# The-Learning-And-Vision-Atelier-LAVA/BUFFER

Hardware: AMD Instinct MI355X
Metric: registration pairs/sec (higher is better)
Workload: dtype f32

## Files before the change

buffer_amd/_lib.py:

```python
import ctypes as C
import os

_HERE = os.path.dirname(os.path.abspath(__file__))
LIB_PATH = os.environ.get("BUF_LIB_PATH") or os.path.join(_HERE, "libbuffer_hip.so")

BUF_OK = 0


class BufferHipError(RuntimeError):
    pass


class buf_grid_t(C.Structure):
    _fields_ = [
        ("ws", C.c_void_p), ("ws_bytes", C.c_size_t),
        ("ns", C.c_int), ("nb", C.c_int),
        ("cells_per_elem", C.c_int64),
        ("radius", C.c_float),
        ("supports", C.c_void_p),
        ("desc", C.c_void_p), ("s_off", C.c_void_p), ("table", C.c_void_p),
        ("sorted", C.c_void_p), ("order", C.c_void_p), ("scan_tmp", C.c_void_p),
    ]


# ... 102 lines not shown
    "buf_sc2_ws_bytes": (_sz, [_vp, _i, _i]),
    "buf_sc2_batched": (_i, [_vp, _vp, _vp, _vp, _vp, _vp, _i, C.c_double, C.c_double, C.c_double, _i, _i, C.c_double, _i, _i,
                             _vp, _vp, _vp, _vp, _vp, _vp, _vp, _vp, _sz, _vp]),
    "buf_clique_ws_bytes": (_sz, [_vp, _i, _i, _i]),
    "buf_clique_batched": (_i, [_vp, _vp, _vp, _vp, _vp, _vp, _i, C.c_double, C.c_double, C.c_double, C.c_double, _i, _i, C.c_double, _i,
                                _i, _vp, _vp, _vp, _vp, _vp, _vp, _vp, _vp, _vp, _vp, _vp, _sz, _vp]),
    "buf_voxel_map_bytes": (_sz, [_i, _i, _i64]),
    "buf_voxel_map_ws_bytes": (_sz, [_i, _i, _i64]),
    "buf_voxel_map_build": (_i, [C.POINTER(buf_voxel_map_t), _vp, _vp, _vp, _i, C.c_double, C.c_double, _i64, _vp, _sz, _vp, _sz, _vp]),
    "buf_voxel_map_export": (_i, [C.POINTER(buf_voxel_map_t), _i, _vp, _vp, _vp, _vp, _vp, _vp]),
    "buf_vgicp_ws_bytes": (_sz, [_i, _i]),
    "buf_vgicp_batched": (_i, [C.POINTER(buf_voxel_map_t), _vp, _vp, _vp, _vp, _i, _i, _vp, _i, C.c_double, C.c_double, _vp, _vp, _vp,
                               _vp, _vp, _vp, _sz, _vp]),
    "buf_match_metrics":(_i, [_vp, _vp, _vp, _i, _i, _vp, _vp, _f, _f, _f, _vp, _vp, _vp]),
    "buf_row_linear": (_i, [_vp, _i, _i, _i, _vp, _vp, _i, _vp, _vp]),
    "buf_segment_instance_norm_ws_bytes": (_sz, [_i, _i]),
    "buf_segment_instance_norm": (_i, [_vp, _i, _i, _vp, _i, _f, _vp, _vp, _sz, _vp]),
    "buf_descriptor_head": (_i, [_vp, _i, _vp, _vp, _vp, _vp]),
    "buf_cost_volume_net": (_i, [_vp, _vp, _i, _vp, _vp, _vp, _vp]),
    "buf_cost_volume_net_gather": (_i, [_vp, _i, _vp, _vp, _i, _vp, _vp, _vp, _vp]),
    "buf_cost_volume_net_w24": (_i, [_vp, _vp, _i, _vp, _vp, _vp, _vp, _vp]),
    "buf_cost_volume_net_w24_gather": (_i, [_vp, _i, _vp, _vp, _i, _vp, _vp, _vp, _vp, _vp]),
    "buf_cost_volume_net_split_safe_w24": (_i, [_vp, _vp, _i, _vp, _vp, _i, _vp, _vp, _vp, _vp, _vp, _vp, _vp, _vp, _vp]),
    "buf_hypotheses_score": (_i, [_vp, _vp, _vp, _vp, _vp, _i, _i, _f, _vp, _vp, _vp, _vp, _vp, _vp]),
    "buf_ransac_ws_bytes": (_sz, [_i]),
    "buf_ransac_kabsch": (_i, [_vp, _vp, _vp, _i, _i, C.c_uint64, _f, _f, _vp, _vp, _vp, _sz, _vp]),
    "buf_ransac_masked_ws_bytes": (_sz, [_i, _i]),
    "buf_ransac_kabsch_masked": (_i, [_vp, _vp, _vp, _i, _i, C.c_uint64, _f, _f, _vp, _vp, _vp, _sz, _vp]),
    "buf_post_refine": (_i, [_vp, _vp, _vp, _i, _f, _i, _vp, _vp, _vp]),
    "buf_recover_poses_ws_bytes": (_sz, [_i, _i, _i]),
    "buf_recover_poses_batched": (_i, [_vp, _vp, _vp, _vp, _vp, _vp, _i, _vp, _i, _f, _i, _f, _f, _f, _i, _vp, _vp, _sz, _vp]),
}


def exported_symbols():
    return sorted(_SIGNATURES)


def lib():
    global _lib
    if _lib is None:
        if not os.path.exists(LIB_PATH):
            raise BufferHipError(
                f"{LIB_PATH} is missing: build it with `python -m buffer_amd.build` "
                "(hipcc --offload-arch=gfx950). buffer_amd has no CPU fallback.")
        import torch
# ... 14 lines not shown
```

buffer_amd/csrc/buffer_hip.hip:

```cpp
#include <stdlib.h>
#include "core.hip"
#include "radius.hip"
#include "icp.hip"
#include "pairstats.hip"
#include "posegraph.hip"
#include "metrics.hip"
#include "subsample.hip"
#include "pointops.hip"
#include "vn.hip"
#include "voxelize.hip"
#include "registration.hip"
#include "convnet.hip"
#include "convnet_h3.hip"
#include "costnet_h3.hip"
#include "preprocess.hip"
#include "convnet_wg.hip"
#include "convnet_w24.hip"
#include "convnet_w24k.hip"
#include "convnet_w24p.hip"
#include "convnet_w24a.hip"
#include "costnet.hip"
#include "costnet_w24.hip"
#include "split_safe.hip"
#include "fpfh.hip"
#include "fgr.hip"
#include "sc2.hip"
#include "clique.hip"
#include "vgicp.hip"
```

buffer_amd/csrc/costnet.hip:

```cpp
#include "common.h"
#include <type_traits>

#define CV_THREADS 256
#define CV_BUF 20480
#define CV_LAYERS 10
#define CV_C32 36
#define CV_C64 68
#define CV_C128 132

typedef float cvx4 __attribute__((ext_vector_type(4)));

#define CV_SCHED_TAIL(NMFMA, NMEM)                                                      \
    _Pragma("unroll") for (int i_ = 0; i_ < (NMFMA); i_++) {                            \
        __builtin_amdgcn_sched_group_barrier(0x008, 1, 0);                              \
        __builtin_amdgcn_sched_group_barrier(0x006, 4, 0);                              \
        __builtin_amdgcn_sched_group_barrier(0x120, ((NMEM) + (NMFMA) - 1) / (NMFMA), 0); \
    }
typedef const __attribute__((address_space(1))) cvx4* cv_gptr;

struct CostNetParams {
    const float* wt[CV_LAYERS];
    const float* bias[CV_LAYERS];
    const long long* s_rows;
    const long long* t_rows;
// ... 240 lines not shown
        int j = lq - (r0 + t);
        j = j < 0 ? j + 20 : j;
        const cvx4 sv = *reinterpret_cast<const cvx4*>(SM + (kq * 20 + j) * CV_C32 + c4 * 4);
        const cvx4 tv = *reinterpret_cast<const cvx4*>(TB + pos * CV_C32 + c4 * 4);
        float* d = X + (kq * 32 + c4 * 4) * CW_CSX + t * CW_RSX + lq;
#pragma unroll
        for (int q = 0; q < 4; q++) d[q * CW_CSX] = fmaxf(sv[q] + tv[q], 0.f);
    }
}

#ifdef CV_STAMP
__device__ long long* cv_stamp_ptr;
#define CV_STAMP_AT(SLOT) if (threadIdx.x == 0) cv_stamp_ptr[(size_t)blockIdx.x * 16 + (SLOT)] = __builtin_amdgcn_s_memtime();
#else
#define CV_STAMP_AT(SLOT)
#endif

#define CW_CS5 72
template <int C, int CS, int USED>
__device__ __forceinline__ void cw24_zero_spare(float* __restrict__ map);
template <int HIN, int RS, int CS, int NTX, int TYPM, int CIN, int RSO, int CSO>
__device__ __forceinline__ void cw24_layer(float* __restrict__ map, const float* __restrict__ wt, const float* __restrict__ bias, int pair, int t);

template <bool W24 = false>
__device__ __forceinline__ void cost_net_body(const float* __restrict__ s_eq, const float* __restrict__ t_eq, const CostNetParams& P,
                                              float* __restrict__ ind_out, float* __restrict__ lds, const float* const* f24 = nullptr)
{
    float* bufA = lds;
    float* bufB = lds;
    float* SP = bufB + CVA_SP;
    float* TP = bufB + CVA_TP;
    float* SM = bufB + CVA_SM;
    float* TB = bufB + CVA_TB;
    const int match = blockIdx.x;
    const int tid = threadIdx.x, lane = tid & (WAVE - 1), li = lane & 15, lk = lane >> 4;
    const int w = __builtin_amdgcn_readfirstlane(tid / WAVE);
    {
        const float* a = s_eq + (P.s_rows ? (size_t)P.s_rows[match] * P.row_floats + P.skip_floats : (size_t)match * 3200);
        const float* b = t_eq + (P.t_rows ? (size_t)P.t_rows[match] * P.row_floats + P.skip_floats : (size_t)match * 3200);
        for (int i = tid; i < 800; i += CV_THREADS) {
            const int c = i / 25, rem = i - c * 25, k = rem / 5, l0 = (rem - k * 5) * 4;
            const cvx4 sv = __builtin_nontemporal_load(reinterpret_cast<const cvx4*>(a + c * P.chan_floats + rem * 4));
            const cvx4 tv = __builtin_nontemporal_load(reinterpret_cast<const cvx4*>(b + c * P.chan_floats + rem * 4));
#pragma unroll
            for (int q = 0; q < 4; q++) {
                const int l = l0 + q;
                SP[(k * 24 + l + 2) * CV_C32 + c] = sv[q];
// ... 11 lines not shown
        int ms = w * 16 + li, mt = ms;
        ms = ms < 60 ? ms : 59;
        mt = mt < 54 ? mt : 53;
        SLoader LS;
        LS.base = SP + ((ms / 20) * 24 + ms % 20) * CV_C32 + lk * 4;
        TLoader LT;
        LT.base = TP + ((mt / 18) * 20 + mt % 18) * CV_C32 + lk * 4;
        cvx4 accS[1][2] = { { (cvx4){ 0.f, 0.f, 0.f, 0.f }, (cvx4){ 0.f, 0.f, 0.f, 0.f } } };
        cvx4 accT[1][2] = { { (cvx4){ 0.f, 0.f, 0.f, 0.f }, (cvx4){ 0.f, 0.f, 0.f, 0.f } } };
        cv_gemm_static<1, 2, 4, 30>(accS, LS, P.wt[0] + (size_t)lane * 4, 2);
        cv_gemm_static<1, 2, 4, 18>(accT, LT, P.wt[0] + (size_t)30 * 2 * 256 + (size_t)lane * 4, 2);
#pragma unroll
        for (int u = 0; u < 2; u++)
#pragma unroll
            for (int r = 0; r < 4; r++) {
                const int m = w * 16 + lk * 4 + r;
                if (m < 60) SM[m * CV_C32 + u * 16 + li] = accS[0][u][r];
                if (m < 54) TB[m * CV_C32 + u * 16 + li] = b0v[u] - accT[0][u][r];
            }
    }
    __syncthreads();
    CV_STAMP_AT(1)

    {
        int lane_ = threadIdx.x & (WAVE - 1);
        asm volatile("" : "+v"(lane_));
        const int li_ = lane_ & 15, lk_ = lane_ >> 4;
        const int p_ = w & 1, kh = w >> 1;
        float* XC = bufB + CVA_XC;
        constexpr unsigned KSTEP = 16u * CW_CSX;
        const __amdgpu_buffer_rsrc_t rs = wg_weights(P.wt[1]);
        const unsigned wp = (unsigned)p_ * (96 * 512) + (unsigned)(12 * kh) * 512;
        const unsigned lofs = lane_ * 16;
        unsigned RA[3][4];
        {
            const unsigned base = (unsigned)(size_t)(__attribute__((address_space(3))) const float*)XC + (unsigned)(12 * kh) * KSTEP;
#pragma unroll
            for (int a = 0; a < 4; a++) RA[0][a] = RA[1][a] = RA[2][a] = base + 4u * (unsigned)(lk_ * CW_CSX + (2 * (li_ >> 3) + a) * CW_RSX + 2 * (li_ & 7));
        }
        const float* bl = kh ? nullptr : P.bias[1] + p_ * 32 + lk_ * 4;
        wgf4 W[2][2];
        wg_first_weights<2, 0, 2>(rs, wp, lofs, 512, W);
        wgf4* slot = reinterpret_cast<wgf4*>(bufB + CVA_XCH) + (size_t)p_ * 8 * WAVE + lane_;
        wgf4 Yown[2][2][3][2][2];
#pragma unroll
        for (int j = 0; j < 4; j++) {
            form_rows_cm(XC, SM, TB, 4 * j);
// ... 12 lines not shown
            }
        }
        __syncthreads();
#pragma unroll
        for (int jj = 0; jj < 2; jj++)
#pragma unroll
            for (int n = 0; n < 2; n++)
                cw_store_tile<18, 2, 16, CW_CS1, false>(Yown[jj][n][0], 2 * kh + jj, 2 * p_ + n, bufA, li_, lk_);
        __syncthreads();
        CV_STAMP_AT(2)
    }
    bool f24_2 = false, f24_4 = false, f24_6 = false;
    if constexpr (W24) { f24_2 = f24[0] != nullptr; f24_4 = f24[1] != nullptr; f24_6 = f24[2] != nullptr; }
    if (W24 && f24_2) {
        if constexpr (W24) {
            cw24_zero_spare<64, CW_CS1, 256>(bufA);
            __syncthreads();
            cw24_layer<16, 16, CW_CS1, 4, 4, 64, 14, CW_CS2>(bufA, f24[0], P.bias[2], w & 1, w >> 1);
        }
    } else
        cw_layer<16, 16, CW_CS1, 2, 64, 2, 2, 0, 14, CW_CS2, false>(bufA, P.wt[2], P.bias[2], w & 1, 2 * (w >> 1));
    __syncthreads();
    CV_STAMP_AT(3)
    cw_layer<14, 14, CW_CS2, 2, 64, 2, 2, 1, 12, CW_CS3, false>(bufA, P.wt[3], P.bias[3], w, 0);
    __syncthreads();
    CV_STAMP_AT(4)
    if (W24 && f24_4) {
        if constexpr (W24) {
            cw24_zero_spare<128, CW_CS3, 144>(bufA);
            __syncthreads();
            cw24_layer<12, 12, CW_CS3, 3, 5, 128, 12, CW_CS3>(bufA, f24[1], P.bias[4], w, 0);
        }
    } else
        cw_layer<12, 12, CW_CS3, 3, 128, 2, 2, 0, 12, CW_CS3, false>(bufA, P.wt[4], P.bias[4], w, 0);
    __syncthreads();
    CV_STAMP_AT(5)
    if (W24 && f24_6) {
        if constexpr (W24) {
            cw_layer<10, 12, CW_CS3, 4, 128, 1, 1, 0, 8, CW_CS5, false>(bufA, P.wt[5], P.bias[5], w, 0);
            __syncthreads();
            CV_STAMP_AT(6)
            cw_layer<8, 8, CW_CS5, 3, 64, 1, 1, 0, 0, CV_C64, true>(bufA, f24[2], P.bias[6], w, 0);
        }
    } else {
        cw_layer<10, 12, CW_CS3, 4, 128, 1, 1, 0, 0, CV_C64, true>(bufA, P.wt[5], P.bias[5], w, 0);
        __syncthreads();
        CV_STAMP_AT(6)
// ... 134 lines not shown
```

buffer_amd/csrc/split_safe.hip:

```cpp
#include "common.h"

extern "C" int buf_cylindrical_net_split_safe_form(const float* x, int npatch, const void* const* wt_split_host, const float* const* wt_wg_host,
                                                   const float* const* bias_host, const int* cin_host, const int* cout_host, const int* relu_host,
                                                   int form, const float* head_params, float* y_or_equi, float* desc, int* status_dev,
                                                   int* flags_ws, void* stream)
{
    BUF_REQUIRE(npatch >= 0, BUF_EINVAL, "buf_cylindrical_net_split_safe: npatch=%d", npatch);
    if (npatch == 0) return BUF_OK;
    BUF_REQUIRE(x && y_or_equi && flags_ws && wt_split_host && wt_wg_host && bias_host && cin_host && cout_host && relu_host, BUF_EINVAL,
                "buf_cylindrical_net_split_safe: null argument");
    BUF_REQUIRE(!head_params || desc, BUF_EINVAL, "buf_cylindrical_net_split_safe: head without desc");
    BUF_REQUIRE(form >= BUF_CYL_FORM_DEFAULT && form <= BUF_CYL_FORM_PASS_SPLIT, BUF_EINVAL,
                "buf_cylindrical_net_split_safe: form=%d (-1: the library's default, 0: K split, 1: pass split)", form);
    if (int rc = buf_cylindrical_net_wg_flags(cin_host, cout_host, relu_host)) return rc;
    hipStream_t s = (hipStream_t)stream;
    BUF_CHECK_HIP(hipMemsetAsync(flags_ws, 0, sizeof(int) * (size_t)npatch, s));
    int relu_split[WG_LAYERS];
    for (int l = 0; l < WG_LAYERS; l++) relu_split[l] = wg_f24_flagged(relu_host[l]) ? (relu_host[l] & 1) : relu_host[l];
    int rc = h3_launch(x, npatch, wt_split_host, bias_host, cin_host, cout_host, relu_split, head_params ? nullptr : y_or_equi, head_params,
                       desc, head_params ? y_or_equi : nullptr, status_dev, stream, flags_ws);
    if (rc) return rc;
    rc = wg_launch(x, npatch, wt_wg_host, bias_host, cin_host, cout_host, relu_host, y_or_equi, flags_ws, stream, form);
    if (rc) return rc;
    if (head_params) {
// ... 58 lines not shown
    if (rc) return rc;
    return cost_net_launch(s_eq, t_eq, m, wt_f32_host, bias_f32_host, s_rows, t_rows, ele_n, ind_out, stream, "buf_cost_volume_net_split_safe", flags_ws);
}

extern "C" int buf_cost_volume_net_split_safe_w24(const float* s_eq, const float* t_eq, int ele_n, const long long* s_rows, const long long* t_rows,
                                                  int m, const void* const* wt_split_host, const float* const* bias_split_host,
                                                  const float* const* wt_f32_host, const float* const* bias_f32_host, const float* const* f24_host,
                                                  float* ind_out, int* status_dev, int* flags_ws, void* stream)
{
    BUF_REQUIRE(m >= 0, BUF_EINVAL, "buf_cost_volume_net_split_safe_w24: m=%d", m);
    if (m == 0) return BUF_OK;
    BUF_REQUIRE(s_eq && t_eq && wt_split_host && bias_split_host && wt_f32_host && bias_f32_host && f24_host && ind_out && flags_ws, BUF_EINVAL,
                "buf_cost_volume_net_split_safe_w24: null argument");
    BUF_REQUIRE((s_rows == nullptr) == (t_rows == nullptr), BUF_EINVAL, "buf_cost_volume_net_split_safe_w24: one row list without the other");
    BUF_REQUIRE(!s_rows || ele_n == 7, BUF_EINVAL, "buf_cost_volume_net_split_safe_w24: ele_n=%d (the kernels are built for ele_n = 7)", ele_n);
    hipStream_t s = (hipStream_t)stream;
    BUF_CHECK_HIP(hipMemsetAsync(flags_ws, 0, sizeof(int) * (size_t)m, s));
    int rc = cost_net_h3_launch(s_eq, t_eq, m, wt_split_host, bias_split_host, s_rows, t_rows, ele_n, ind_out, status_dev, stream,
                                "buf_cost_volume_net_split_safe_w24", flags_ws);
    if (rc) return rc;
    return cost_net_w24_launch(s_eq, t_eq, m, wt_f32_host, bias_f32_host, f24_host, s_rows, t_rows, ele_n, ind_out, stream,
                               "buf_cost_volume_net_split_safe_w24", flags_ws);
}
```

buffer_amd/ops.py:

```python
import ctypes as C
import time
import os
import numpy as np
import torch

from . import _lib
from ._lib import buf_grid_t, check


def _stream():
    return C.c_void_p(torch.cuda.current_stream().cuda_stream)


def _dev(t, dtype, what):
    if not isinstance(t, torch.Tensor) or not t.is_cuda:
        raise _lib.BufferHipError(f"{what}: expected a tensor in device memory (buffer_amd has no CPU path)")
    if t.dtype != dtype:
        t = t.to(dtype)
    return t.contiguous()


def _ptr(t):
    return C.c_void_p(t.data_ptr()) if t is not None else C.c_void_p(0)

# ... 1078 lines not shown
        f24 = COST_F24_DEFAULT
    if f24 is True:
        f24 = 'all'
    if f24 is False:
        f24 = 'off'
    if f24 not in COST_F24_PARTS:
        raise ValueError(f"f24 = {f24!r}: one of 'all', 'l2', 'l4', 'l6', 'off'")
    return COST_F24_PARTS[f24]


def cost_f24_filters(layers, parts):
    sets = []
    for l in (2, 4, 6):
        if l not in parts:
            sets.append(None)
            continue
        w = layers[l][0]
        assert tuple(w.shape[2:]) == (3, 1, 3), w.shape
        w2d = np.ascontiguousarray(w[:, :, :, 0, :])
        sets.append(winograd_tile_weights(w2d, ng=1) if l == 6 else winograd_f24_tile_weights(w2d))
    return sets


class CostVolumeNet:

    def __init__(self, layers, device, f24=None):
        assert len(layers) == 10
        self.parts = cost_f24_parts(f24)
        self.wt24 = [None if a is None else torch.from_numpy(a).to(device) for a in cost_f24_filters(layers, self.parts)]
        self._fp = (C.c_void_p * 3)(*[None if t is None else t.data_ptr() for t in self.wt24])
        self.wt, self.bias = [], []
        for i, (w, b) in enumerate(layers):
            cout, cin = w.shape[0], w.shape[1]
            b = np.asarray(b, np.float32)
            if i == 0:
                assert tuple(w.shape) == (32, 32, 3, 3, 3), w.shape
                tiled = np.concatenate([mfma_tile_weights(m, lk_major=True) for m in separate_cost_layer0(w)])
                self.wt.append(torch.from_numpy(tiled).to(device))
                self.bias.append(torch.from_numpy(np.ascontiguousarray(b)).to(device))
                continue
            if i == 1:
                assert tuple(w.shape) == (64, 32, 3, 3, 3), w.shape
                w2d = np.ascontiguousarray(np.transpose(w, (0, 3, 1, 2, 4)).reshape(64, 96, 3, 3))
                self.wt.append(torch.from_numpy(winograd_tile_weights(w2d, ng=_lib.lib().buf_cost_winograd_group(1))).to(device))
                self.bias.append(torch.from_numpy(np.ascontiguousarray(b)).to(device))
                continue
            if 2 <= i <= 5:
                assert tuple(w.shape[2:]) == (3, 1, 3), w.shape
                tiled = winograd_tile_weights(np.ascontiguousarray(w[:, :, :, 0, :]), ng=_lib.lib().buf_cost_winograd_group(i))
                self.wt.append(torch.from_numpy(tiled).to(device))
                self.bias.append(torch.from_numpy(np.ascontiguousarray(b)).to(device))
                continue
            wt = np.transpose(w, (2, 3, 4, 1, 0)).reshape(-1, cout)
            if i == 9:
                wt = np.concatenate([wt, np.zeros((wt.shape[0], 32 - cout), np.float32)], 1)
                b = np.concatenate([b, np.zeros(32 - cout, np.float32)])
            self.wt.append(torch.from_numpy(mfma_tile_weights(np.ascontiguousarray(wt, dtype=np.float32), lk_major=True)).to(device))
            self.bias.append(torch.from_numpy(np.ascontiguousarray(b)).to(device))
        self._wp = (C.c_void_p * 10)(*[t.data_ptr() for t in self.wt])
        self._bp = (C.c_void_p * 10)(*[t.data_ptr() for t in self.bias])

    def __call__(self, s_eq, t_eq):
        L = _lib.lib()
        s_eq, t_eq = s_eq.contiguous(), t_eq.contiguous()
        m = s_eq.shape[0]
        out = torch.empty((m,), dtype=torch.float32, device=s_eq.device)
        if self.parts:
            check(L.buf_cost_volume_net_w24(_ptr(s_eq), _ptr(t_eq), m, self._wp, self._bp, self._fp, _ptr(out), _stream()),
                  "buf_cost_volume_net_w24")
            return out
        check(L.buf_cost_volume_net(_ptr(s_eq), _ptr(t_eq), m, self._wp, self._bp, _ptr(out), _stream()),
              "buf_cost_volume_net")
        return out

    def gathered(self, equi, s_rows, t_rows):
        L = _lib.lib()
        equi = _dev(equi, torch.float32, "CostVolumeNet.gathered")
        if equi.dim() != 4 or tuple(equi.shape[1:]) != (32, 7, 20):
            raise _lib.BufferHipError(f"CostVolumeNet.gathered: expected [rows,32,7,20] maps, got {tuple(equi.shape)}")
        s_rows, t_rows = _dev(s_rows, torch.int64, "s_rows"), _dev(t_rows, torch.int64, "t_rows")
        m = int(s_rows.shape[0])
        out = torch.empty((m,), dtype=torch.float32, device=equi.device)
        if self.parts:
            check(L.buf_cost_volume_net_w24_gather(_ptr(equi), 7, _ptr(s_rows), _ptr(t_rows), m, self._wp, self._bp, self._fp, _ptr(out),
                                                   _stream()), "buf_cost_volume_net_w24_gather")
            return out
        check(L.buf_cost_volume_net_gather(_ptr(equi), 7, _ptr(s_rows), _ptr(t_rows), m, self._wp, self._bp, _ptr(out), _stream()),
              "buf_cost_volume_net_gather")
        return out


class CostVolumeNetSplit:

    def __init__(self, layers, device, f24=None):
        assert len(layers) == 10
        self.parts = cost_f24_parts(f24)
        mats = []
        w0 = layers[0][0]
        assert tuple(w0.shape) == (32, 32, 3, 3, 3), w0.shape
        ws, wt = separate_cost_layer0(w0)
        mats.append((np.transpose(ws.reshape(15, 32, 32), (2, 1, 0)), 2))
        mats.append((np.transpose(wt.reshape(9, 32, 32), (2, 1, 0)), 2))
        w1 = layers[1][0]
        assert tuple(w1.shape) == (64, 32, 3, 3, 3), w1.shape
        mats.append((np.transpose(w1, (0, 3, 1, 2, 4)).reshape(64, 96, 9), 2))
        for i in range(2, 9):
            w = layers[i][0]
            assert tuple(w.shape[2:]) == (3, 1, 3), w.shape
            mats.append((np.ascontiguousarray(w[:, :, :, 0, :]).reshape(w.shape[0], w.shape[1], 9), 2 if i < 7 else 1))
        w9 = layers[9][0]
        assert tuple(w9.shape) == (20, 32, 2, 1, 2), w9.shape
        mats.append((np.ascontiguousarray(w9[:, :, :, 0, :]).reshape(20, 32, 4), 1))
        self.wt = [torch.from_numpy(split_tile_gemm(m, nt).view(np.int16)).to(device) for m, nt in mats]
        self.bias = []
        for i, (_, b) in enumerate(layers):
            b = np.asarray(b, np.float32)
            if i == 9:
                b = np.concatenate([b, np.zeros(32 - b.shape[0], np.float32)])
            self.bias.append(torch.from_numpy(np.ascontiguousarray(b)).to(device))
        self.status = torch.zeros(1, dtype=torch.int32, device=device)
        self._wp = (C.c_void_p * 11)(*[t.data_ptr() for t in self.wt])
        self._bp = (C.c_void_p * 10)(*[t.data_ptr() for t in self.bias])
        self.safe = not os.environ.get('BUF_SPLIT_UNSAFE')
        self.f32 = CostVolumeNet(layers, device, f24=f24) if self.safe else None
        self.last_flags = None

    def _safe(self, s_eq, t_eq, s_rows, t_rows, m, dev):
        L = _lib.lib()
        out = torch.empty((m,), dtype=torch.float32, device=dev)
        self.last_flags = torch.empty((max(m, 1),), dtype=torch.int32, device=dev)
        if self.parts:
            check(L.buf_cost_volume_net_split_safe_w24(_ptr(s_eq), _ptr(t_eq), 7, _ptr(s_rows), _ptr(t_rows), m, self._wp, self._bp, self.f32._wp,
                                                       self.f32._bp, self.f32._fp, _ptr(out), _ptr(self.status), _ptr(self.last_flags), _stream()),
                  "buf_cost_volume_net_split_safe_w24")
            return out
        check(L.buf_cost_volume_net_split_safe(_ptr(s_eq), _ptr(t_eq), 7, _ptr(s_rows), _ptr(t_rows), m, self._wp, self._bp, self.f32._wp,
                                               self.f32._bp, _ptr(out), _ptr(self.status), _ptr(self.last_flags), _stream()),
              "buf_cost_volume_net_split_safe")
        return out

    def __call__(self, s_eq, t_eq):
        L = _lib.lib()
        s_eq, t_eq = s_eq.contiguous(), t_eq.contiguous()
        m = s_eq.shape[0]
        if self.safe:
            return self._safe(s_eq, t_eq, None, None, m, s_eq.device)
        out = torch.empty((m,), dtype=torch.float32, device=s_eq.device)
        check(L.buf_cost_volume_net_split(_ptr(s_eq), _ptr(t_eq), m, self._wp, self._bp, _ptr(out), _ptr(self.status), _stream()),
              "buf_cost_volume_net_split")
        return out

    def gathered(self, equi, s_rows, t_rows):
        L = _lib.lib()
# ... 21 lines not shown
```

buffer_amd/registration.py:

```python
import numpy as np

from . import ops
from .patch_embedder import _fold_bn


class CostVolume:

    def __init__(self, W, device, azi_n=20, arith='f32', f24=None):
        if arith not in ('f32', 'split'):
            raise ValueError(f"cnn_arith must be 'f32' or 'split', got {arith!r}")
        if azi_n != 20:
            raise NotImplementedError(f'CostVolume: the fused kernel is built for azi_n = 20 (got {azi_n})')
        self.azi_n = azi_n
        p = 'Inlier.conv.ops'
        layers = []
        for i, bn in ((0, 1), (3, 4), (6, 7), (9, 10), (12, 13), (15, 16), (18, 19), (21, 22), (24, 25)):
            layers.append(_fold_bn(W[f'{p}.{i}.weight'], W[f'{p}.{i}.bias'], W[f'{p}.{bn}.running_mean'], W[f'{p}.{bn}.running_var']))
        layers.append((np.asarray(W[f'{p}.27.weight'], np.float32), np.asarray(W[f'{p}.27.bias'], np.float32)))
        self.fused = ops.CostVolumeNetSplit(layers, device, f24=f24) if arith == 'split' else ops.CostVolumeNet(layers, device, f24=f24)

    def __call__(self, d1, d2):
        if tuple(d1.shape[1:]) != (32, 5, 20) or d1.shape != d2.shape:
            raise ValueError(f'CostVolume: expected two [M,32,5,20] maps, got {tuple(d1.shape)} and {tuple(d2.shape)}')
        return self.fused(d1, d2)

    def gathered(self, equi, s_rows, t_rows):
        return self.fused.gathered(equi, s_rows, t_rows)
```

include/buffer_hip.h:

```cpp
#ifndef BUFFER_HIP_H
#define BUFFER_HIP_H
#include <stddef.h>
#include <stdint.h>
#ifdef __cplusplus
extern "C" {
#endif

#define BUF_OK            0
#define BUF_EINVAL       -1
#define BUF_EHIP         -2
#define BUF_EWORKSPACE   -3
#define BUF_ECAPACITY    -4
#define BUF_ENODEVICE    -5

const char* buf_last_error(void);
int         buf_version(void);
int         buf_device_count(void);
#define BUF_TIMED_GRID_QUERY 0
#define BUF_TIMED_CYL_NET    1
#define BUF_TIMED_COST_NET   2
#define BUF_TIMED_SELECT_PATCHES 3
#define BUF_TIMED_PATCH_VOXELIZE 4
#define BUF_TIMED_FPS            5
#define BUF_TIMED_NN1            6
// ... 150 lines not shown
                                       const float* head_params, float* y_or_equi, float* desc, int* status_dev, int* flags_ws, void* stream);

int     buf_cylindrical_net_split_safe_form(const float* x, int npatch, const void* const* wt_split_host, const float* const* wt_wg_host,
                                            const float* const* bias_host, const int* cin_host, const int* cout_host, const int* relu_host,
                                            int form, const float* head_params, float* y_or_equi, float* desc, int* status_dev, int* flags_ws,
                                            void* stream);
int     buf_cylindrical_net_split_safe_all(const float* x, int npatch, const void* const* wt_split_host, const float* const* wt_wg_host,
                                           const float* const* bias_host, const int* cin_host, const int* cout_host, const int* relu_host,
                                           const float* const* wt24_host, const float* head_params, float* y_or_equi, float* desc,
                                           int* status_dev, int* flags_ws, void* stream);

int     buf_descriptor_head(const float* y, int npatch, const float* params, float* desc, float* equi, void* stream);

int     buf_cost_winograd_group(int layer);
int     buf_cost_volume_net(const float* s_eq, const float* t_eq, int m, const float* const* wt_host,
                            const float* const* bias_host, float* ind_out, void* stream);
int     buf_cost_volume_net_gather(const float* equi, int ele_n, const long long* s_rows, const long long* t_rows, int m,
                                   const float* const* wt_host, const float* const* bias_host, float* ind_out, void* stream);
int     buf_cost_volume_net_w24(const float* s_eq, const float* t_eq, int m, const float* const* wt_host, const float* const* bias_host,
                                const float* const* f24_host, float* ind_out, void* stream);
int     buf_cost_volume_net_w24_gather(const float* equi, int ele_n, const long long* s_rows, const long long* t_rows, int m,
                                       const float* const* wt_host, const float* const* bias_host, const float* const* f24_host,
                                       float* ind_out, void* stream);

long long buf_split_gemm_count(int cout, int cin, int ntaps, int nt);
int     buf_split_tile_gemm(const float* w_host, int cout, int cin, int ntaps, int nt, unsigned short* out_host);
int     buf_cost_volume_net_split(const float* s_eq, const float* t_eq, int m, const void* const* wt_host,
                                  const float* const* bias_host, float* ind_out, int* status_dev, void* stream);
int     buf_cost_volume_net_split_gather(const float* equi, int ele_n, const long long* s_rows, const long long* t_rows, int m,
                                         const void* const* wt_host, const float* const* bias_host, float* ind_out,
                                         int* status_dev, void* stream);
int     buf_cost_volume_net_split_safe(const float* s_eq, const float* t_eq, int ele_n, const long long* s_rows, const long long* t_rows,
                                       int m, const void* const* wt_split_host, const float* const* bias_split_host,
                                       const float* const* wt_f32_host, const float* const* bias_f32_host, float* ind_out,
                                       int* status_dev, int* flags_ws, void* stream);
int     buf_cost_volume_net_split_safe_w24(const float* s_eq, const float* t_eq, int ele_n, const long long* s_rows, const long long* t_rows,
                                           int m, const void* const* wt_split_host, const float* const* bias_split_host,
                                           const float* const* wt_f32_host, const float* const* bias_f32_host, const float* const* f24_host,
                                           float* ind_out, int* status_dev, int* flags_ws, void* stream);

int     buf_hypotheses_score(const float* ind, const float* ss_kpts, const float* tt_kpts, const float* ss_R,
                             const float* tt_R, int m, int azi_n, float inlier_th, float* R_out, float* t_out,
                             int* inlier_num, int* best_out, unsigned char* best_mask, void* stream);
size_t  buf_ransac_ws_bytes(int nhyp);
int     buf_ransac_kabsch(const float* src, const float* tgt, const int* corr, int ncorr, int nhyp,
                          unsigned long long seed, float max_dist, float edge_similarity, float* T_out,
                          int* info_out, void* ws, size_t ws_bytes, void* stream);
size_t  buf_ransac_masked_ws_bytes(int m, int nhyp);
int     buf_ransac_kabsch_masked(const float* src, const float* tgt, const unsigned char* mask, int m, int nhyp,
                                 unsigned long long seed, float max_dist, float edge_similarity, float* T_out,
                                 int* info_out, void* ws, size_t ws_bytes, void* stream);
int     buf_post_refine(const float* T_init, const float* src, const float* tgt, int m, float inlier_threshold,
                        int iters, float* T_out, int* info_out, void* stream);
size_t  buf_recover_poses_ws_bytes(int m_total, int nb, int nhyp);
int     buf_recover_poses_batched(const float* ind, const float* ss_kpts, const float* tt_kpts, const float* ss_R, const float* tt_R,
                                  const int* seg_host, int nb, const unsigned long long* seeds_host, int azi_n, float inlier_th,
                                  int nhyp, float max_dist, float edge_similarity, float refine_threshold, int refine_iters,
                                  float* poses_out, void* ws, size_t ws_bytes, void* stream);

size_t  buf_voxel_downsample_ws_bytes(int n, int64_t max_cells);
int     buf_voxel_downsample(const void* pts, const void* normals, int is_f64, int n, double voxel_size, double* out_pts,
                             double* out_normals, int* out_m_host, int64_t max_cells, void* ws, size_t ws_bytes, void* stream);
// ... 127 lines not shown
```

Measured before the change: 175.3.

## Add Winograd F(2x4) paths for cost-volume layers 1 and 3

Adds a w24b cost-net kernel that computes layer 1 (a 3x3x3 conv folded into a 2D conv over 96 channels, with the input plane formed per depth slice) and layer 3 with Winograd F(2x4) tiles. Layer 3 also gets an F(2x2) tail for the leftover rows. It becomes the default when f24 is unset, and the goal is fewer multiply-adds in these direct convolutions. The cost is extra transform arithmetic, extra LDS plane rebuilding and syncs, register pressure, and small floating-point differences.

Result: faster. 177.3, median of 6 (+1.1%).

```diff
diff --git a/buffer_amd/_lib.py b/buffer_amd/_lib.py
--- a/buffer_amd/_lib.py
+++ b/buffer_amd/_lib.py
@@ -148,6 +148,9 @@
     "buf_cost_volume_net_w24": (_i, [_vp, _vp, _i, _vp, _vp, _vp, _vp, _vp]),
     "buf_cost_volume_net_w24_gather": (_i, [_vp, _i, _vp, _vp, _i, _vp, _vp, _vp, _vp, _vp]),
     "buf_cost_volume_net_split_safe_w24": (_i, [_vp, _vp, _i, _vp, _vp, _i, _vp, _vp, _vp, _vp, _vp, _vp, _vp, _vp, _vp]),
+    "buf_cost_volume_net_w24b": (_i, [_vp, _vp, _i, _vp, _vp, _vp, _vp, _vp]),
+    "buf_cost_volume_net_w24b_gather": (_i, [_vp, _i, _vp, _vp, _i, _vp, _vp, _vp, _vp, _vp]),
+    "buf_cost_volume_net_split_safe_w24b": (_i, [_vp, _vp, _i, _vp, _vp, _i, _vp, _vp, _vp, _vp, _vp, _vp, _vp, _vp, _vp]),
     "buf_hypotheses_score": (_i, [_vp, _vp, _vp, _vp, _vp, _i, _i, _f, _vp, _vp, _vp, _vp, _vp, _vp]),
     "buf_ransac_ws_bytes": (_sz, [_i]),
     "buf_ransac_kabsch": (_i, [_vp, _vp, _vp, _i, _i, C.c_uint64, _f, _f, _vp, _vp, _vp, _sz, _vp]),
diff --git a/buffer_amd/csrc/buffer_hip.hip b/buffer_amd/csrc/buffer_hip.hip
--- a/buffer_amd/csrc/buffer_hip.hip
+++ b/buffer_amd/csrc/buffer_hip.hip
@@ -21,6 +21,7 @@
 #include "convnet_w24a.hip"
 #include "costnet.hip"
 #include "costnet_w24.hip"
+#include "costnet_w24b.hip"
 #include "split_safe.hip"
 #include "fpfh.hip"
 #include "fgr.hip"
diff --git a/buffer_amd/csrc/costnet.hip b/buffer_amd/csrc/costnet.hip
--- a/buffer_amd/csrc/costnet.hip
+++ b/buffer_amd/csrc/costnet.hip
@@ -286,7 +286,11 @@
 template <int HIN, int RS, int CS, int NTX, int TYPM, int CIN, int RSO, int CSO>
 __device__ __forceinline__ void cw24_layer(float* __restrict__ map, const float* __restrict__ wt, const float* __restrict__ bias, int pair, int t);
 
-template <bool W24 = false>
+__device__ __forceinline__ void cw24b_layer1(float* __restrict__ lds, const float* __restrict__ wt, const float* __restrict__ bias, int w);
+__device__ __forceinline__ void cw24b_layer3(float* __restrict__ map, const float* __restrict__ wt24, const float* __restrict__ wt22,
+                                             const float* __restrict__ bias, int w);
+
+template <bool W24 = false, bool W24B = false>
 __device__ __forceinline__ void cost_net_body(const float* __restrict__ s_eq, const float* __restrict__ t_eq, const CostNetParams& P,
                                               float* __restrict__ ind_out, float* __restrict__ lds, const float* const* f24 = nullptr)
 {
@@ -344,7 +348,14 @@
     __syncthreads();
     CV_STAMP_AT(1)
 
-    {
+    bool f24_1 = false, f24_3 = false;
+    if constexpr (W24B) { f24_1 = f24[3] != nullptr; f24_3 = f24[4] != nullptr; }
+    if (W24B && f24_1) {
+        if constexpr (W24B) {
+            cw24b_layer1(lds, f24[3], P.bias[1], w);
+            CV_STAMP_AT(2)
+        }
+    } else {
         int lane_ = threadIdx.x & (WAVE - 1);
         asm volatile("" : "+v"(lane_));
         const int li_ = lane_ & 15, lk_ = lane_ >> 4;
@@ -403,7 +414,10 @@
         cw_layer<16, 16, CW_CS1, 2, 64, 2, 2, 0, 14, CW_CS2, false>(bufA, P.wt[2], P.bias[2], w & 1, 2 * (w >> 1));
     __syncthreads();
     CV_STAMP_AT(3)
-    cw_layer<14, 14, CW_CS2, 2, 64, 2, 2, 1, 12, CW_CS3, false>(bufA, P.wt[3], P.bias[3], w, 0);
+    if (W24B && f24_3) {
+        if constexpr (W24B) cw24b_layer3(bufA, f24[4], P.wt[3], P.bias[3], w);
+    } else
+        cw_layer<14, 14, CW_CS2, 2, 64, 2, 2, 1, 12, CW_CS3, false>(bufA, P.wt[3], P.bias[3], w, 0);
     __syncthreads();
     CV_STAMP_AT(4)
     if (W24 && f24_4) {
diff --git a/buffer_amd/csrc/costnet_w24b.hip b/buffer_amd/csrc/costnet_w24b.hip
--- /dev/null
+++ b/buffer_amd/csrc/costnet_w24b.hip
@@ -0,0 +1,281 @@
+#include "common.h"
+
+#ifndef CWB_RS1
+#define CWB_RS1 24
+#define CWB_CS1 450
+#endif
+static_assert(32 * CWB_CS1 <= CVA_SM, "the plane ends in front of the layer-0 maps");
+static_assert(17 * CWB_RS1 + 4 * 3 + 6 <= CWB_CS1 && CWB_RS1 % 2 == 0 && CWB_CS1 % 2 == 0, "the last window stays inside the channel; ds_read_b64");
+static_assert(64 * CW_CS1 <= CV_BUF, "layer 1's output map");
+
+struct CostNetW24BParams {
+    CostNetParams P;
+    const float* f24[5];
+};
+
+__device__ __forceinline__ void cw24b_form_plane(float* __restrict__ X, const float* __restrict__ SM, const float* __restrict__ TB, int kq)
+{
+    for (int i = threadIdx.x; i < 324 * 8; i += CV_THREADS) {
+        const int c4 = i & 7, pos = i >> 3, n = pos / 18, lq = pos - n * 18;
+        int j = lq - n;
+        j = j < 0 ? j + 20 : j;
+        const cvx4 sv = *reinterpret_cast<const cvx4*>(SM + (kq * 20 + j) * CV_C32 + c4 * 4);
+        const cvx4 tv = *reinterpret_cast<const cvx4*>(TB + (kq * 18 + lq) * CV_C32 + c4 * 4);
+        float* d = X + c4 * 4 * CWB_CS1 + n * CWB_RS1 + lq;
+#pragma unroll
+        for (int q = 0; q < 4; q++) d[q * CWB_CS1] = fmaxf(sv[q] + tv[q], 0.f);
+    }
+}
+
+template <unsigned KSTEP>
+__device__ __forceinline__ void cw24b_round_add(unsigned (&RA)[4], __amdgpu_buffer_rsrc_t rs, unsigned wp, unsigned wp_after, unsigned lofs4, unsigned lofs2,
+                                                int niter, unsigned pstride, const float* __restrict__ bias_lane, wgf4 (&W4)[2][2], wgf2 (&W2)[2][2],
+                                                wgf4 (&Y)[2][2][4])
+{
+    using std::integral_constant;
+    wgf2 D[2][6];
+    wgf4 bv[2];
+#pragma unroll
+    for (int n = 0; n < 2; n++) bv[n] = bias_lane ? *reinterpret_cast<const wgf4*>(bias_lane + n * 16) : (wgf4){ 0.f, 0.f, 0.f, 0.f };
+    wgf4 acc[2][6];
+    float zero = 0.f;
+    asm volatile("" : "+v"(zero));
+    auto run = [&](auto ic) __attribute__((always_inline)) {
+        constexpr int I = decltype(ic)::value;
+        constexpr int INEXT = I == 3 ? 0 : I + 1;
+#pragma unroll
+        for (int n = 0; n < 2; n++)
+#pragma unroll
+            for (int j = 0; j < 6; j++) acc[n][j] = (I == 1 && j == 1) ? bv[n] : (wgf4){ zero, zero, zero, zero };
+        constexpr int ICHAIN = (INEXT != 0 && wg_chains(I)) ? INEXT : -1;
+        w24_pass<I, wg_chains(I - 1), ICHAIN, KSTEP>(RA, rs, wp + I * pstride, INEXT == 0 ? wp_after : wp + (I + 1) * pstride, lofs4, lofs2, niter, W4, W2, acc, D);
+        __builtin_amdgcn_sched_barrier(0);
+#pragma unroll
+        for (int n = 0; n < 2; n++) {
+            wgf4 f[4];
+#pragma unroll
+            for (int r = 0; r < 4; r++) {
+                const float p = acc[n][1][r] + acc[n][2][r], q = acc[n][1][r] - acc[n][2][r];
+                const float t = acc[n][3][r] + acc[n][4][r], d = acc[n][3][r] - acc[n][4][r];
+                f[0][r] = acc[n][0][r] + p + t;
+                f[1][r] = __builtin_fmaf(2.f, d, q);
+                f[2][r] = __builtin_fmaf(4.f, t, p);
+                f[3][r] = __builtin_fmaf(8.f, d, q) + acc[n][5][r];
+            }
+#pragma unroll
+            for (int v = 0; v < 4; v++) {
+                if constexpr (I <= 2) Y[n][0][v] += f[v];
+                if constexpr (I == 1) Y[n][1][v] += f[v];
+                if constexpr (I >= 2) Y[n][1][v] -= f[v];
+                if constexpr (I <= 2) asm volatile("" : "+v"(Y[n][0][v]));
+                if constexpr (I >= 1) asm volatile("" : "+v"(Y[n][1][v]));
+            }
+        }
+    };
+    run(integral_constant<int, 0>{});
+    run(integral_constant<int, 1>{});
+    run(integral_constant<int, 2>{});
+    run(integral_constant<int, 3>{});
+}
+
+__device__ __forceinline__ void cw24b_layer1(float* __restrict__ lds, const float* __restrict__ wt, const float* __restrict__ bias, int w)
+{
+    float* X = lds + CVA_XC;
+    const float* SM = lds + CVA_SM;
+    const float* TB = lds + CVA_TB;
+    constexpr unsigned KSTEP = 16u * CWB_CS1;
+    int lane = threadIdx.x & (WAVE - 1);
+    asm volatile("" : "+v"(lane));
+    const int lk = lane >> 4;
+    const int pair = w & 1, t = w >> 1;
+    unsigned RA[4];
+    {
+        const unsigned base = (unsigned)(size_t)(__attribute__((address_space(3))) const float*)X;
+        const int li = lane & 15, ty = 4 * t + (li >> 2), tx = li & 3;
+#pragma unroll
+        for (int a = 0; a < 4; a++) RA[a] = base + 4u * (unsigned)(lk * CWB_CS1 + (2 * ty + a) * CWB_RS1 + 4 * tx);
+    }
+    const __amdgpu_buffer_rsrc_t rs = wg_weights(wt);
+    const unsigned pstride = 24u * W24_WSTRIDE;
+    const unsigned wp0 = (unsigned)pair * 4 * pstride;
+    const unsigned lofs4 = lane * 16, lofs2 = lane * 8;
+    const float* bv = bias + (2 * pair) * 16 + lk * 4;
+    wgf4 W4[2][2];
+    wgf2 W2[2][2];
+#pragma unroll
+    for (int n = 0; n < 2; n++)
+#pragma unroll
+        for (int k = 0; k < 2; k++) {
+            W4[n][k] = wg_ldw(rs, wp0 + k * W24_WSTRIDE + n * 256, lofs4);
+            W2[n][k] = w24_ldw2(rs, wp0 + k * W24_WSTRIDE + 512 + n * 128, lofs2);
+        }
+    wgf4 Y[2][2][4];
+    {
+        float zero = 0.f;
+        asm volatile("" : "+v"(zero));
+#pragma unroll
+        for (int q = 0; q < 16; q++) Y[q >> 3][(q >> 2) & 1][q & 3] = (wgf4){ zero, zero, zero, zero };
+    }
+#pragma unroll 1
+    for (int k = 0; k < 3; k++) {
+        cw24b_form_plane(X, SM, TB, k);
+        __syncthreads();
+        const unsigned wp = wp0 + 8u * k * W24_WSTRIDE;
+        cw24b_round_add<KSTEP>(RA, rs, wp, k < 2 ? wp + 8u * W24_WSTRIDE : wp0, lofs4, lofs2, 2, pstride, k == 0 ? bv : nullptr, W4, W2, Y);
+        __syncthreads();
+    }
+    int lane_s = threadIdx.x & (WAVE - 1);
+    asm volatile("" : "+v"(lane_s));
+    const int li = lane_s & 15, ty = 4 * t + (li >> 2), tx = li & 3;
+#pragma unroll
+    for (int n = 0; n < 2; n++) {
+        float* p = lds + ((2 * pair + n) * 16 + (lane_s >> 4) * 4) * CW_CS1 + 2 * ty * 16 + 4 * tx;
+#pragma unroll
+        for (int u = 0; u < 2; u++)
+#pragma unroll
+            for (int r = 0; r < 4; r++)
+                *reinterpret_cast<wgf4*>(p + r * CW_CS1 + u * 16) = (wgf4){ fmaxf(Y[n][u][0][r], 0.f), fmaxf(Y[n][u][1][r], 0.f), fmaxf(Y[n][u][2][r], 0.f), fmaxf(Y[n][u][3][r], 0.f) };
+    }
+    __syncthreads();
+}
+
+__device__ __forceinline__ void cw24b_layer3(float* __restrict__ map, const float* __restrict__ wt24, const float* __restrict__ wt22,
+                                             const float* __restrict__ bias, int w)
+{
+    constexpr int HIN = 14, RS = 14, CS = CW_CS2, NTX = 3, TYPM = 5, CIN = 64, RSO = 12, CSO = CW_CS3, k4 = CIN / 4;
+    static_assert((2 * (TYPM - 1) + 3) * RS + 4 * (NTX - 1) + 6 <= HIN * RS && RS % 2 == 0 && CS % 2 == 0, "the last F(2x4) window ends inside its row");
+    constexpr unsigned KSTEP = 16u * CS;
+    int lane = threadIdx.x & (WAVE - 1);
+    asm volatile("" : "+v"(lane));
+    const int lk = lane >> 4;
+    const unsigned base = (unsigned)(size_t)(__attribute__((address_space(3))) const float*)map;
+    unsigned RA[4];
+    {
+        const int li = lane & 15, q = li / NTX;
+        int ty = q, tx = li - q * NTX;
+        if (q >= TYPM) { ty = 0; tx = 0; }
+#pragma unroll
+        for (int a = 0; a < 4; a++) RA[a] = base + 4u * (unsigned)(lk * CS + (2 * ty + a) * RS + 4 * tx);
+    }
+    const unsigned lofs4 = lane * 16, lofs2 = lane * 8;
+    const float* bv = bias + (2 * w) * 16 + lk * 4;
+    wgf4 Y[2][2][4];
+    {
+        const __amdgpu_buffer_rsrc_t rs = wg_weights(wt24);
+        const unsigned pstride = (unsigned)(k4 * W24_WSTRIDE);
+        const unsigned wp = (unsigned)w * 4 * pstride;
+        wgf4 W4[2][2];
+        wgf2 W2[2][2];
+#pragma unroll
+        for (int n = 0; n < 2; n++)
+#pragma unroll
+            for (int k = 0; k < 2; k++) {
+                W4[n][k] = wg_ldw(rs, wp + k * W24_WSTRIDE + n * 256, lofs4);
+                W2[n][k] = w24_ldw2(rs, wp + k * W24_WSTRIDE + 512 + n * 128, lofs2);
+            }
+        w24_round<false, KSTEP>(RA, rs, wp, wp, lofs4, lofs2, k4 >> 2, pstride, bv, W4, W2, Y);
+    }
+    wgf4 Y2[2][3][2][2];
+    {
+        unsigned RB[3][4];
+        const int li = lane & 15, q = li / 6;
+        int ty = 4 + q, tx = li - q * 6;
+        if (q >= 2) { ty = 0; tx = 0; }
+#pragma unroll
+        for (int a = 0; a < 4; a++) RB[0][a] = RB[1][a] = RB[2][a] = base + 4u * (unsigned)(lk * CS + (2 * ty + a) * RS + 2 * tx);
+        const __amdgpu_buffer_rsrc_t rs = wg_weights(wt22);
+        const unsigned wp = (unsigned)w * (CIN * 2 * 256);
+        wgf4 W[2][2];
+        wg_first_weights<2, 0, 2>(rs, wp, lofs4, 512, W);
+        wg_round<2, 0, 1, KSTEP, true>(RB, rs, wp, wp, lofs4, k4 >> 2, 512, (unsigned)(k4 * 512), bv, W, Y2);
+    }
+    __syncthreads();
+    int lane_s = threadIdx.x & (WAVE - 1);
+    asm volatile("" : "+v"(lane_s));
+    const int li = lane_s & 15;
+    {
+        const int q = li / NTX, tx = li - q * NTX;
+        if (q < TYPM) {
+#pragma unroll
+            for (int n = 0; n < 2; n++) {
+                float* p = map + ((2 * w + n) * 16 + (lane_s >> 4) * 4) * CSO + 2 * q * RSO + 4 * tx;
+#pragma unroll
+                for (int u = 0; u < 2; u++)
+#pragma unroll
+                    for (int r = 0; r < 4; r++)
+                        *reinterpret_cast<wgf4*>(p + r * CSO + u * RSO) = (wgf4){ fmaxf(Y[n][u][0][r], 0.f), fmaxf(Y[n][u][1][r], 0.f), fmaxf(Y[n][u][2][r], 0.f), fmaxf(Y[n][u][3][r], 0.f) };
+            }
+        }
+    }
+    if (li >= 6 && li < 12) {
+#pragma unroll
+        for (int n = 0; n < 2; n++) {
+            float* p = map + ((2 * w + n) * 16 + (lane_s >> 4) * 4) * CSO + 10 * RSO + 2 * (li - 6);
+#pragma unroll
+            for (int u = 0; u < 2; u++)
+#pragma unroll
+                for (int r = 0; r < 4; r++)
+                    *reinterpret_cast<wgf2*>(p + r * CSO + u * RSO) = (wgf2){ fmaxf(Y2[n][0][u][0][r], 0.f), fmaxf(Y2[n][0][u][1][r], 0.f) };
+        }
+    }
+}
+
+__global__ void __launch_bounds__(CV_THREADS, 2) k_cost_net_w24b(const float* __restrict__ s_eq, const float* __restrict__ t_eq, CostNetW24BParams Q,
+                                                             float* __restrict__ ind_out)
+{
+    extern __shared__ float lds[];
+    cost_net_body<true, true>(s_eq, t_eq, Q.P, ind_out, lds, Q.f24);
+}
+
+__global__ void __launch_bounds__(CV_THREADS, 2) k_cost_net_w24b_rerun(const float* __restrict__ s_eq, const float* __restrict__ t_eq, CostNetW24BParams Q,
+                                                                   float* __restrict__ ind_out)
+{
+    extern __shared__ float lds[];
+    if (Q.P.only_if[blockIdx.x] == 0) return;
+    cost_net_body<true, true>(s_eq, t_eq, Q.P, ind_out, lds, Q.f24);
+}
+
+static int cost_net_w24b_launch(const float* s_eq, const float* t_eq, int m, const float* const* wt_host, const float* const* bias_host,
+                                const float* const* f24_host, const long long* s_rows, const long long* t_rows, int ele_n, float* ind_out,
+                                void* stream, const char* who, const int* only_if = nullptr)
+{
+    CostNetW24BParams Q;
+    if (int rc = cost_net_params(Q.P, wt_host, bias_host, s_rows, t_rows, ele_n, only_if, who)) return rc;
+    for (int i = 0; i < 5; i++) Q.f24[i] = f24_host[i];
+    size_t lds = sizeof(float) * CV_BUF;
+    static LdsGrant grant, grant_rerun;
+    if (int rc = only_if ? grant_dynamic_lds((const void*)k_cost_net_w24b_rerun, lds, grant_rerun) : grant_dynamic_lds((const void*)k_cost_net_w24b, lds, grant)) return rc;
+    TimedSpan span;
+    bool timed = !only_if && timing_begin((hipStream_t)stream, &span, 2.0 * cost_net_macs_per_match * m, BUF_TIMED_COST_NET);
+#ifdef CV_STAMP
+    long long* stamps = nullptr;
+    if (int rc = cv_stamp_begin(m, &stamps)) return rc;
+#endif
+    if (only_if) k_cost_net_w24b_rerun<<<m, CV_THREADS, lds, (hipStream_t)stream>>>(s_eq, t_eq, Q, ind_out);
+    else k_cost_net_w24b<<<m, CV_THREADS, lds, (hipStream_t)stream>>>(s_eq, t_eq, Q, ind_out);
+    if (timed) timing_end((hipStream_t)stream, &span);
+    BUF_LAUNCH_CHECK();
+#ifdef CV_STAMP
+    if (int rc = cv_stamp_end(m, stamps, stream, "k_cost_net_w24b")) return rc;
+#endif
+    return BUF_OK;
+}
+
+extern "C" int buf_cost_volume_net_w24b(const float* s_eq, const float* t_eq, int m, const float* const* wt_host, const float* const* bias_host,
+                                        const float* const* f24_host, float* ind_out, void* stream)
+{
+    BUF_REQUIRE(m >= 0, BUF_EINVAL, "buf_cost_volume_net_w24b: m=%d", m);
+    if (m == 0) return BUF_OK;
+    BUF_REQUIRE(s_eq && t_eq && wt_host && bias_host && f24_host && ind_out, BUF_EINVAL, "buf_cost_volume_net_w24b: null argument");
+    return cost_net_w24b_launch(s_eq, t_eq, m, wt_host, bias_host, f24_host, nullptr, nullptr, 7, ind_out, stream, "buf_cost_volume_net_w24b");
+}
+
+extern "C" int buf_cost_volume_net_w24b_gather(const float* equi, int ele_n, const long long* s_rows, const long long* t_rows, int m,
+                                               const float* const* wt_host, const float* const* bias_host, const float* const* f24_host,
+                                               float* ind_out, void* stream)
+{
+    BUF_REQUIRE(m >= 0 && ele_n == 7, BUF_EINVAL, "buf_cost_volume_net_w24b_gather: m=%d ele_n=%d (the kernel is built for ele_n = 7)", m, ele_n);
+    if (m == 0) return BUF_OK;
+    BUF_REQUIRE(equi && s_rows && t_rows && wt_host && bias_host && f24_host && ind_out, BUF_EINVAL, "buf_cost_volume_net_w24b_gather: null argument");
+    return cost_net_w24b_launch(equi, equi, m, wt_host, bias_host, f24_host, s_rows, t_rows, ele_n, ind_out, stream, "buf_cost_volume_net_w24b_gather");
+}
diff --git a/buffer_amd/csrc/split_safe.hip b/buffer_amd/csrc/split_safe.hip
--- a/buffer_amd/csrc/split_safe.hip
+++ b/buffer_amd/csrc/split_safe.hip
@@ -104,3 +104,23 @@
     return cost_net_w24_launch(s_eq, t_eq, m, wt_f32_host, bias_f32_host, f24_host, s_rows, t_rows, ele_n, ind_out, stream,
                                "buf_cost_volume_net_split_safe_w24", flags_ws);
 }
+
+extern "C" int buf_cost_volume_net_split_safe_w24b(const float* s_eq, const float* t_eq, int ele_n, const long long* s_rows, const long long* t_rows,
+                                                   int m, const void* const* wt_split_host, const float* const* bias_split_host,
+                                                   const float* const* wt_f32_host, const float* const* bias_f32_host, const float* const* f24_host,
+                                                   float* ind_out, int* status_dev, int* flags_ws, void* stream)
+{
+    BUF_REQUIRE(m >= 0, BUF_EINVAL, "buf_cost_volume_net_split_safe_w24b: m=%d", m);
+    if (m == 0) return BUF_OK;
+    BUF_REQUIRE(s_eq && t_eq && wt_split_host && bias_split_host && wt_f32_host && bias_f32_host && f24_host && ind_out && flags_ws, BUF_EINVAL,
+                "buf_cost_volume_net_split_safe_w24b: null argument");
+    BUF_REQUIRE((s_rows == nullptr) == (t_rows == nullptr), BUF_EINVAL, "buf_cost_volume_net_split_safe_w24b: one row list without the other");
+    BUF_REQUIRE(!s_rows || ele_n == 7, BUF_EINVAL, "buf_cost_volume_net_split_safe_w24b: ele_n=%d (the kernels are built for ele_n = 7)", ele_n);
+    hipStream_t s = (hipStream_t)stream;
+    BUF_CHECK_HIP(hipMemsetAsync(flags_ws, 0, sizeof(int) * (size_t)m, s));
+    int rc = cost_net_h3_launch(s_eq, t_eq, m, wt_split_host, bias_split_host, s_rows, t_rows, ele_n, ind_out, status_dev, stream,
+                                "buf_cost_volume_net_split_safe_w24b", flags_ws);
+    if (rc) return rc;
+    return cost_net_w24b_launch(s_eq, t_eq, m, wt_f32_host, bias_f32_host, f24_host, s_rows, t_rows, ele_n, ind_out, stream,
+                                "buf_cost_volume_net_split_safe_w24b", flags_ws);
+}
diff --git a/buffer_amd/ops.py b/buffer_amd/ops.py
--- a/buffer_amd/ops.py
+++ b/buffer_amd/ops.py
@@ -1124,13 +1124,49 @@
     return sets
 
 
+COST_F24B_DEFAULT = 'all'
+COST_F24B_PARTS = {'all': (1, 3), 'l1': (1,), 'l3': (3,), 'off': ()}
+
+
+def cost_f24b_parts(f24, f24b):
+    if f24b is None:
+        f24b = COST_F24B_DEFAULT if f24 is None else 'off'
+    if f24b is True:
+        f24b = 'all'
+    if f24b is False:
+        f24b = 'off'
+    if f24b not in COST_F24B_PARTS:
+        raise ValueError(f"f24b = {f24b!r}: one of 'all', 'l1', 'l3', 'off'")
+    return COST_F24B_PARTS[f24b]
+
+
+def cost_f24b_filters(layers, parts):
+    sets = []
+    for l in (1, 3):
+        if l not in parts:
+            sets.append(None)
+            continue
+        w = layers[l][0]
+        if l == 1:
+            assert tuple(w.shape) == (64, 32, 3, 3, 3), w.shape
+            w2d = np.ascontiguousarray(np.transpose(w, (0, 3, 1, 2, 4)).reshape(64, 96, 3, 3))
+        else:
+            assert tuple(w.shape[2:]) == (3, 1, 3), w.shape
+            w2d = np.ascontiguousarray(w[:, :, :, 0, :])
+        sets.append(winograd_f24_tile_weights(w2d))
+    return sets
+
+
 class CostVolumeNet:
 
-    def __init__(self, layers, device, f24=None):
+    def __init__(self, layers, device, f24=None, f24b=None):
         assert len(layers) == 10
         self.parts = cost_f24_parts(f24)
+        self.parts_b = cost_f24b_parts(f24, f24b)
         self.wt24 = [None if a is None else torch.from_numpy(a).to(device) for a in cost_f24_filters(layers, self.parts)]
         self._fp = (C.c_void_p * 3)(*[None if t is None else t.data_ptr() for t in self.wt24])
+        self.wt24b = [None if a is None else torch.from_numpy(a).to(device) for a in cost_f24b_filters(layers, self.parts_b)]
+        self._fpb = (C.c_void_p * 5)(*[None if t is None else t.data_ptr() for t in self.wt24 + self.wt24b])
         self.wt, self.bias = [], []
         for i, (w, b) in enumerate(layers):
             cout, cin = w.shape[0], w.shape[1]
@@ -1167,6 +1203,10 @@
         s_eq, t_eq = s_eq.contiguous(), t_eq.contiguous()
         m = s_eq.shape[0]
         out = torch.empty((m,), dtype=torch.float32, device=s_eq.device)
+        if self.parts_b:
+            check(L.buf_cost_volume_net_w24b(_ptr(s_eq), _ptr(t_eq), m, self._wp, self._bp, self._fpb, _ptr(out), _stream()),
+                  "buf_cost_volume_net_w24b")
+            return out
         if self.parts:
             check(L.buf_cost_volume_net_w24(_ptr(s_eq), _ptr(t_eq), m, self._wp, self._bp, self._fp, _ptr(out), _stream()),
                   "buf_cost_volume_net_w24")
@@ -1183,6 +1223,10 @@
         s_rows, t_rows = _dev(s_rows, torch.int64, "s_rows"), _dev(t_rows, torch.int64, "t_rows")
         m = int(s_rows.shape[0])
         out = torch.empty((m,), dtype=torch.float32, device=equi.device)
+        if self.parts_b:
+            check(L.buf_cost_volume_net_w24b_gather(_ptr(equi), 7, _ptr(s_rows), _ptr(t_rows), m, self._wp, self._bp, self._fpb, _ptr(out),
+                                                    _stream()), "buf_cost_volume_net_w24b_gather")
+            return out
         if self.parts:
             check(L.buf_cost_volume_net_w24_gather(_ptr(equi), 7, _ptr(s_rows), _ptr(t_rows), m, self._wp, self._bp, self._fp, _ptr(out),
                                                    _stream()), "buf_cost_volume_net_w24_gather")
@@ -1194,9 +1238,10 @@
 
 class CostVolumeNetSplit:
 
-    def __init__(self, layers, device, f24=None):
+    def __init__(self, layers, device, f24=None, f24b=None):
         assert len(layers) == 10
         self.parts = cost_f24_parts(f24)
+        self.parts_b = cost_f24b_parts(f24, f24b)
         mats = []
         w0 = layers[0][0]
         assert tuple(w0.shape) == (32, 32, 3, 3, 3), w0.shape
@@ -1224,13 +1269,18 @@
         self._wp = (C.c_void_p * 11)(*[t.data_ptr() for t in self.wt])
         self._bp = (C.c_void_p * 10)(*[t.data_ptr() for t in self.bias])
         self.safe = not os.environ.get('BUF_SPLIT_UNSAFE')
-        self.f32 = CostVolumeNet(layers, device, f24=f24) if self.safe else None
+        self.f32 = CostVolumeNet(layers, device, f24=f24, f24b=f24b) if self.safe else None
         self.last_flags = None
 
     def _safe(self, s_eq, t_eq, s_rows, t_rows, m, dev):
         L = _lib.lib()
         out = torch.empty((m,), dtype=torch.float32, device=dev)
         self.last_flags = torch.empty((max(m, 1),), dtype=torch.int32, device=dev)
+        if self.parts_b:
+            check(L.buf_cost_volume_net_split_safe_w24b(_ptr(s_eq), _ptr(t_eq), 7, _ptr(s_rows), _ptr(t_rows), m, self._wp, self._bp, self.f32._wp,
+                                                        self.f32._bp, self.f32._fpb, _ptr(out), _ptr(self.status), _ptr(self.last_flags), _stream()),
+                  "buf_cost_volume_net_split_safe_w24b")
+            return out
         if self.parts:
             check(L.buf_cost_volume_net_split_safe_w24(_ptr(s_eq), _ptr(t_eq), 7, _ptr(s_rows), _ptr(t_rows), m, self._wp, self._bp, self.f32._wp,
                                                        self.f32._bp, self.f32._fp, _ptr(out), _ptr(self.status), _ptr(self.last_flags), _stream()),
diff --git a/buffer_amd/registration.py b/buffer_amd/registration.py
--- a/buffer_amd/registration.py
+++ b/buffer_amd/registration.py
@@ -6,7 +6,7 @@
 
 class CostVolume:
 
-    def __init__(self, W, device, azi_n=20, arith='f32', f24=None):
+    def __init__(self, W, device, azi_n=20, arith='f32', f24=None, f24b=None):
         if arith not in ('f32', 'split'):
             raise ValueError(f"cnn_arith must be 'f32' or 'split', got {arith!r}")
         if azi_n != 20:
@@ -17,7 +17,8 @@
         for i, bn in ((0, 1), (3, 4), (6, 7), (9, 10), (12, 13), (15, 16), (18, 19), (21, 22), (24, 25)):
             layers.append(_fold_bn(W[f'{p}.{i}.weight'], W[f'{p}.{i}.bias'], W[f'{p}.{bn}.running_mean'], W[f'{p}.{bn}.running_var']))
         layers.append((np.asarray(W[f'{p}.27.weight'], np.float32), np.asarray(W[f'{p}.27.bias'], np.float32)))
-        self.fused = ops.CostVolumeNetSplit(layers, device, f24=f24) if arith == 'split' else ops.CostVolumeNet(layers, device, f24=f24)
+        cls = ops.CostVolumeNetSplit if arith == 'split' else ops.CostVolumeNet
+        self.fused = cls(layers, device, f24=f24, f24b=f24b)
 
     def __call__(self, d1, d2):
         if tuple(d1.shape[1:]) != (32, 5, 20) or d1.shape != d2.shape:
diff --git a/include/buffer_hip.h b/include/buffer_hip.h
--- a/include/buffer_hip.h
+++ b/include/buffer_hip.h
@@ -196,6 +196,11 @@
 int     buf_cost_volume_net_w24_gather(const float* equi, int ele_n, const long long* s_rows, const long long* t_rows, int m,
                                        const float* const* wt_host, const float* const* bias_host, const float* const* f24_host,
                                        float* ind_out, void* stream);
+int     buf_cost_volume_net_w24b(const float* s_eq, const float* t_eq, int m, const float* const* wt_host, const float* const* bias_host,
+                                 const float* const* f24_host, float* ind_out, void* stream);
+int     buf_cost_volume_net_w24b_gather(const float* equi, int ele_n, const long long* s_rows, const long long* t_rows, int m,
+                                        const float* const* wt_host, const float* const* bias_host, const float* const* f24_host,
+                                        float* ind_out, void* stream);
 
 long long buf_split_gemm_count(int cout, int cin, int ntaps, int nt);
 int     buf_split_tile_gemm(const float* w_host, int cout, int cin, int ntaps, int nt, unsigned short* out_host);
@@ -212,6 +217,10 @@
                                            int m, const void* const* wt_split_host, const float* const* bias_split_host,
                                            const float* const* wt_f32_host, const float* const* bias_f32_host, const float* const* f24_host,
                                            float* ind_out, int* status_dev, int* flags_ws, void* stream);
+int     buf_cost_volume_net_split_safe_w24b(const float* s_eq, const float* t_eq, int ele_n, const long long* s_rows, const long long* t_rows,
+                                            int m, const void* const* wt_split_host, const float* const* bias_split_host,
+                                            const float* const* wt_f32_host, const float* const* bias_f32_host, const float* const* f24_host,
+                                            float* ind_out, int* status_dev, int* flags_ws, void* stream);
 
 int     buf_hypotheses_score(const float* ind, const float* ss_kpts, const float* tt_kpts, const float* ss_R,
                              const float* tt_R, int m, int azi_n, float inlier_th, float* R_out, float* t_out,
```
